# JunkyByte/easy_ViTPose

Hardware: NVIDIA H100
Metric: person-crops/sec ViT-B 256x192 bf16 (higher is better)
Workload: dtype bf16

## Files before the change

easy_vitpose_b200/csrc/engine.cu:

```cuda
#include <cuda.h>
#include <cuda_runtime.h>

#include <algorithm>
#include <cmath>
#include <cstdarg>
#include <cstdio>
#include <cstdlib>
#include <cstring>
#include <map>
#include <mutex>
#include <string>
#include <vector>

#include "../../include/vitpose_b200.h"
#include "attention.cuh"
#include "chain.cuh"
#include "decode.cuh"
#include "draw.cuh"
#include "expert_gemm.cuh"
#include "gemm.cuh"
#include "pointwise.cuh"
#include "preprocess.cuh"
#include "qkv_attention.cuh"
#include "track.cuh"
// ... 81 lines not shown
static cudaError_t launch_k(void (*kern)(KArgs...), dim3 grid, dim3 block, size_t smem, cudaStream_t st, Args&&... args) {
  cudaLaunchConfig_t cfg;
  memset(&cfg, 0, sizeof(cfg));
  cfg.gridDim = grid; cfg.blockDim = block; cfg.dynamicSmemBytes = smem; cfg.stream = st;
  cudaLaunchAttribute at[1];
  at[0].id = cudaLaunchAttributeProgrammaticStreamSerialization;
  at[0].val.programmaticStreamSerializationAllowed = 1;
  cfg.attrs = at; cfg.numAttrs = g_pdl ? 1 : 0;
  return cudaLaunchKernelEx(&cfg, kern, std::forward<Args>(args)...);
}

constexpr int kMaxDevices = 64;
struct DeviceState {
  int sms = 0;
  bool attn_attr = false;
  unsigned gemm_attr = 0;
  unsigned expert_attr = 0;
};
static DeviceState g_devs[kMaxDevices];
static DeviceState* cur_dev() {
  int d = 0;
  if (cudaGetDevice(&d) != cudaSuccess || d < 0 || d >= kMaxDevices) d = 0;
  return &g_devs[d];
}
static int num_sms() { return cur_dev()->sms; }


constexpr int gemm_slot(int bn, int epi) {
  return (epi == EPI_BF16_GELU_ERF ? 3 : epi) * 5 + (bn == 256 ? 0 : bn == 128 ? 1 : bn == 144 ? 2 : bn == 32 ? 3 : 4);
}
static_assert(gemm_slot(192, EPI_F32_ADD) < 32, "gemm_attr has 32 bits");

template <int BN, int EPI>
static int gemm_launch_t(const CUtensorMap& ta, const CUtensorMap& tw, const CUtensorMap& tout, const GemmParams& p, cudaStream_t st) {
  using Cfg = GemmCfg<BN, EPI>;
  auto kern = gemm_bf16_wgmma<BN, EPI>;
  DeviceState* ds = cur_dev();
  if (ds->sms == 0) return fail(VPB_ERR_STATE, "gemm: device not initialised (device_check)");
  constexpr unsigned slot = 1u << gemm_slot(BN, EPI);
  if (!(ds->gemm_attr & slot)) {
    CU_TRY(cudaFuncSetAttribute(kern, cudaFuncAttributeMaxDynamicSharedMemorySize, Cfg::SMEM_BYTES));
    ds->gemm_attr |= slot;
  }
  const bool deconv = (EPI == EPI_BF16_RELU_UP);
  const int num_m = deconv ? p.M / (p.up_tr * p.up_tw) : (p.M + GEMM_BM - 1) / GEMM_BM;
  const int tiles = num_m * (deconv ? 4 : (p.N + BN - 1) / BN);
  const int grid = tiles < ds->sms ? tiles : ds->sms;
  CU_TRY(launch_k(kern, dim3(grid), dim3(GEMM_THREADS), Cfg::SMEM_BYTES, st, ta, tw, tout, p));
  return VPB_OK;
}
static int gemm_launch(int bn, int epi, const CUtensorMap& ta, const CUtensorMap& tw, const CUtensorMap& tout, const GemmParams& p,
                       cudaStream_t st) {
  if (p.K % GEMM_BK != 0 || p.K <= 0) return fail(VPB_ERR_ARG, "gemm: K=%d must be a positive multiple of 64", p.K);
  if (epi_uses_tma(epi) && (p.N % (epi == EPI_F32_ADD ? 32 : 64) != 0 || p.bias == nullptr))
    return fail(VPB_ERR_ARG, "gemm: TMA epilogue wants N %% 64 == 0 (N %% 32 == 0 for the fp32 one) and a bias");
#define VPB_CASE(BN_, EPI_) \
  if (bn == BN_ && epi == EPI_) return gemm_launch_t<BN_, EPI_>(ta, tw, tout, p, st);
  VPB_CASE(256, EPI_BF16) VPB_CASE(192, EPI_BF16) VPB_CASE(128, EPI_BF16)
  VPB_CASE(256, EPI_BF16_GELU) VPB_CASE(192, EPI_BF16_GELU) VPB_CASE(128, EPI_BF16_GELU)
  VPB_CASE(256, EPI_BF16_GELU_ERF) VPB_CASE(192, EPI_BF16_GELU_ERF) VPB_CASE(128, EPI_BF16_GELU_ERF)
  VPB_CASE(256, EPI_F32_ADD) VPB_CASE(192, EPI_F32_ADD) VPB_CASE(128, EPI_F32_ADD)
  VPB_CASE(256, EPI_BF16_RELU_UP)
  VPB_CASE(32, EPI_F32_NCHW) VPB_CASE(144, EPI_F32_NCHW)
#undef VPB_CASE
  return fail(VPB_ERR_ARG, "gemm: no kernel for BN=%d epilogue=%d", bn, epi);
}

constexpr int kExpertWidths[5] = {192, 128, 96, 64, 32};
static int expert_width(int P) {
  for (int w : kExpertWidths)
    if (P % w == 0) return w;
  return 0;
}
template <int BN>
static int expert_launch_t(const CUtensorMap& ta, const CUtensorMap& tw, const ExpertParams& p, cudaStream_t st) {
  using Cfg = TileCfg<BN, false>;
  auto kern = gemm_expert_segments<BN>;
  DeviceState* ds = cur_dev();
  if (ds->sms == 0) return fail(VPB_ERR_STATE, "expert gemm: device not initialised (device_check)");
  constexpr unsigned slot = 1u << (BN / 32);
// ... 195 lines not shown
};
struct HeadW {
  int K = 0, n_final = 0;
  LinearW dc1, dc2, fin;
  CUtensorMap m_fin_w;
};
struct Segment { int head, count; };
static bool operator==(const Segment& a, const Segment& b) { return a.head == b.head && a.count == b.count; }
struct vpb_engine {
  vpb_config cfg;
  int D, depth, heads, K, maxB;
  int num_kheads = 1, P = 0, Kmax = 0, expert_bn = 0;
  std::vector<HeadW> hw;
  bool finalized = false;
  int stop_after = 0;
  Profiler prof;
  struct CachedGraph { bool mixed; std::vector<Segment> segs; bool affine; cudaGraphExec_t exec; unsigned long long used; };
  std::vector<CachedGraph> graph_cache;
  unsigned long long graph_clock = 0;
  bool use_graph = true;
  bool l2_persist = true;
  size_t l2_window_bytes = 0;
  std::vector<cudaStream_t> l2_streams;
  float* g_kpts = nullptr;
  int32_t *g_idx = nullptr, *g_org = nullptr, *g_offs = nullptr;
  float* g_cs = nullptr;
  double* mat_stage = nullptr;
  float* cs_stage = nullptr;
  int32_t *pp_org = nullptr, *pp_offs = nullptr, *pp_status = nullptr;
  uint8_t* frame_stage[2] = {nullptr, nullptr};
  size_t frame_cap[2] = {0, 0};
  int32_t* bbox_stage[2] = {nullptr, nullptr};
  bool flip = false, flip_heads = false;
// ... 699 lines not shown
      else fuse_ln(p, e->lnf_g, e->lnf_b);
      e->prof.begin(KC_GEMM_FC2, st);
      int bn;
      const CUtensorMap* wm;
      VPB_TRY(pick_tile(b.fc2, M, &bn, &wm));
      p.rmw = resid_rmw(e->resid_rmw);
      VPB_TRY(gemm_launch(bn, EPI_F32_ADD, e->m_hid, *wm, e->o_x, p, st));
      e->prof.end(st);
    }
    if (stop == 8) return VPB_OK;
  }
  if (stop == 9) return VPB_OK;
  return standalone_ln(e->lnf_g, e->lnf_b);
}

static int head(vpb_engine* e, int B, float* d_heat, cudaStream_t st, int j = 0, int c0 = 0, int ch_stride = 0) {
  const int D = e->D;
  const int stop = e->stop_after;
  const HeadW& h = e->hw[j];
  CUtensorMap feat = e->m_feat_nhwc, d1 = e->m_d1_nhwc, d2 = e->m_d2;
  if (c0 > 0) {
    VPB_TRY(make_map_nhwc(&feat, e->xn + static_cast<size_t>(c0) * 192 * D, B, 16, 12, D, 8, 12));
    VPB_TRY(make_map_nhwc(&d1, e->d1 + static_cast<size_t>(c0) * 768 * 256, B, 32, 24, 256, 16, 8));
    VPB_TRY(make_map(&d2, e->d2 + static_cast<size_t>(c0) * 3072 * 256, static_cast<uint64_t>(B) * 3072, 256, 256, 128));
  }
  {
    GemmParams p = gp(B * 192, 256, 4 * D, h.dc1.b, e->d1 + static_cast<size_t>(c0) * 768 * 256, 256);
    p.up_h = 16; p.up_w = 12; p.up_tr = 8; p.up_tw = 12; p.up_c = D;
    e->prof.begin(KC_GEMM_DECONV, st);
    VPB_TRY(gemm_launch(256, EPI_BF16_RELU_UP, feat, *h.dc1.tile_map(256), e->m_xn, p, st));
    e->prof.end(st);
  }
  if (stop == 11) return VPB_OK;
  {
    GemmParams p = gp(B * 768, 256, 1024, h.dc2.b, e->d2 + static_cast<size_t>(c0) * 3072 * 256, 256);
    p.up_h = 32; p.up_w = 24; p.up_tr = 16; p.up_tw = 8; p.up_c = 256;
    e->prof.begin(KC_GEMM_DECONV, st);
    VPB_TRY(gemm_launch(256, EPI_BF16_RELU_UP, d1, *h.dc2.tile_map(256), e->m_xn, p, st));
    e->prof.end(st);
  }
  if (stop == 12) return VPB_OK;
  {
    GemmParams p = gp(B * 3072, h.n_final, 256, h.fin.b, d_heat, 0);
    p.n_valid = h.K; p.pix = 3072; p.ch_stride = ch_stride;
    e->prof.begin(KC_GEMM_FINAL, st);
    VPB_TRY(gemm_launch(h.n_final, EPI_F32_NCHW, d2, h.m_fin_w, d2, p, st));
    e->prof.end(st);
  }
  return VPB_OK;
}

static int apply_l2_policy(vpb_engine* e, cudaStream_t st) {
  if (!e->l2_persist || e->l2_window_bytes == 0) return VPB_OK;
  for (cudaStream_t s : e->l2_streams) if (s == st) return VPB_OK;
  cudaStreamAttrValue v;
// ... 73 lines not shown
  if (e->flip && 2 * batch > e->maxB)
    return fail(VPB_ERR_ARG, "batch %d: with flip test on a call takes at most max_batch / 2 = %d crops (max_batch=%d)", batch, e->maxB / 2, e->maxB);
  return VPB_OK;
}

extern "C" int vpb_forward(vpb_engine* e, const float* d_crops, int32_t batch, float* d_heatmaps, void* stream) {
  VPB_TRY(check_ready(e, batch));
  DeviceGuard dev_guard(e);
  if (!d_crops || !d_heatmaps) return fail(VPB_ERR_ARG, "vpb_forward: null pointer");
  cudaStream_t st = static_cast<cudaStream_t>(stream);
  VPB_TRY(apply_l2_policy(e, st));
  WsScope ws(e, st);
  VPB_TRY(ws.begin(batch));
  VPB_TRY(patch_gather(e, d_crops, batch, batch, st));
  VPB_TRY(backbone(e, batch, st));
  if (!(e->stop_after && e->stop_after <= 10)) VPB_TRY(head(e, batch, d_heatmaps, st));
  return ws.end();
}

extern "C" int vpb_forward_features(vpb_engine* e, const float* d_crops, int32_t batch, float* d_features, void* stream) {
  VPB_TRY(check_ready(e, batch));
  DeviceGuard dev_guard(e);
  if (!d_crops || !d_features) return fail(VPB_ERR_ARG, "vpb_forward_features: null pointer");
  cudaStream_t st = static_cast<cudaStream_t>(stream);
  WsScope ws(e, st);
  VPB_TRY(ws.begin(batch));
  VPB_TRY(patch_gather(e, d_crops, batch, batch, st));
  VPB_TRY(backbone(e, batch, st));
  const long long tot = static_cast<long long>(batch) * e->D * 192;
  tokens_to_nchw<<<cdiv(tot, 256), 256, 0, st>>>(e->xn, d_features, batch, e->D);
  CU_TRY(cudaGetLastError());
// ... 14 lines not shown
}
extern "C" int vpb_decode(const float* d_heatmaps, int32_t n, int32_t k, const int32_t* d_org_wh, float* d_kpts, int32_t* d_idx,
                          int32_t wrap_batch, void* stream) {
  return decode_launch(d_heatmaps, n, k, d_org_wh, nullptr, d_kpts, d_idx, wrap_batch, stream);
}
extern "C" int vpb_head(vpb_engine* e, const float* d_features, int32_t batch, float* d_heatmaps, void* stream) {
  VPB_TRY(check_ready(e, batch));
  DeviceGuard dev_guard(e);
  if (!d_features || !d_heatmaps) return fail(VPB_ERR_ARG, "vpb_head: null pointer");
  cudaStream_t st = static_cast<cudaStream_t>(stream);
  const long long tot = static_cast<long long>(batch) * e->D * 192;
  WsScope ws(e, st);
  VPB_TRY(ws.begin(0));
  nchw_to_tokens<<<cdiv(tot, 256), 256, 0, st>>>(d_features, e->xn, batch, e->D);
  CU_TRY(cudaGetLastError());
  VPB_TRY(head(e, batch, d_heatmaps, st));
  return ws.end();
}
extern "C" int vpb_flip_back(const float* d_in, int32_t n, int32_t k, const int32_t* d_perm, int32_t shift, float* d_out, void* stream) {
  if (!d_in || !d_out || !d_perm || d_in == d_out) return fail(VPB_ERR_ARG, "vpb_flip_back: null or aliased pointers");
  if (n < 0 || k < 1) return fail(VPB_ERR_ARG, "vpb_flip_back: n=%d k=%d", n, k);
  if (n == 0) return VPB_OK;
  const long long tot = static_cast<long long>(n) * k * 3072;
  flip_back_heatmaps<<<cdiv(tot, 256), 256, 0, static_cast<cudaStream_t>(stream)>>>(d_in, d_out, d_perm, n, k, shift);
  CU_TRY(cudaGetLastError());
  return VPB_OK;
}
static bool gauss_taps(int ksize, GaussTaps& tp) {
  if (ksize < 1 || ksize > 2 * MAX_RADIUS + 1 || ksize % 2 == 0) return false;
  const int r = ksize / 2;
  if (ksize <= 9) {
// ... 85 lines not shown
  return out;
}

static int row_stride(const vpb_engine* e, bool mixed) { return mixed ? e->Kmax : e->K; }

static int heads_enqueue(vpb_engine* e, const Source* src, const std::vector<Segment>& segs, int n, int kstride, const int32_t* d_org_wh,
                         const int32_t* d_offs_yx, const float* d_cs, float* d_kpts, int32_t* d_idx, float* heat, cudaStream_t st) {
  const std::vector<Segment> msegs = model_segments(e, segs);
  const int nb = model_crops(e, n);
  if (src) VPB_TRY(gather(e, *src, n, nb, st));
  VPB_TRY(backbone(e, nb, st, (msegs.size() == 1 && msegs[0].head == 0) ? nullptr : &msegs));
  if (e->stop_after && e->stop_after <= 10) return VPB_OK;
  float* raw = e->flip ? e->heat : heat;
  int c0 = 0;
  for (const Segment& sg : msegs) {
    VPB_TRY(head(e, sg.count, raw + static_cast<size_t>(c0) * kstride * 3072, st, sg.head, c0, kstride));
    c0 += sg.count;
  }
  if (e->stop_after) return VPB_OK;
  c0 = 0;
  for (const Segment& sg : segs) {
    const size_t m0 = static_cast<size_t>(c0) * kstride * 3072;
    const int K = e->hw[sg.head].K;
    if (e->flip) VPB_TRY(flip_average(e, raw + m0, sg.count, K, e->flip_perm + perm_offset(e, sg.head), kstride, n, heat + m0, st));
    DecodeParams p;
    p.heatmaps = heat + m0; p.org_wh = d_cs ? nullptr : d_org_wh + 2 * c0; p.offs_yx = (d_offs_yx && !d_cs) ? d_offs_yx + 2 * c0 : nullptr;
    p.kpts = d_kpts + static_cast<size_t>(c0) * kstride * 3; p.idx = d_idx ? d_idx + static_cast<size_t>(c0) * kstride : nullptr;
    p.n = sg.count; p.k = K; p.kstride = kstride;
    p.wrap_batch = d_cs ? 1 : 0;
    p.cs32 = d_cs ? d_cs + 4 * c0 : nullptr;
    e->prof.begin(KC_DECODE, st);
// ... 19 lines not shown
  return VPB_OK;
}

static_assert(2 * VPB_MAX_SEGMENTS <= EXPERT_MAX_SEGMENTS, "a flip-test call's crops and mirror images fit the expert GEMM's table");
constexpr size_t kMaxMixedGraphs = 16;

static void drop_graphs(vpb_engine* e) {
  for (auto& g : e->graph_cache) if (g.exec) cudaGraphExecDestroy(g.exec);
  e->graph_cache.clear();
}

static int heads_core_locked(vpb_engine* e, const Source& src, const std::vector<Segment>& segs, bool mixed, int n, const int32_t* d_org_wh,
                             const int32_t* d_offs_yx, float* d_kpts, int32_t* d_idx, float* d_heatmaps, cudaStream_t st) {
  float* heat = d_heatmaps ? d_heatmaps : e->heat;
  const int ks = row_stride(e, mixed);
  if (!e->use_graph || e->prof.on || e->stop_after || st == nullptr || stream_is_capturing(st))
    return heads_enqueue(e, &src, segs, n, ks, d_org_wh, d_offs_yx, src.cs, d_kpts, d_idx, heat, st);
  const bool affine = src.cs != nullptr;
  vpb_engine::CachedGraph* g = nullptr;
  for (auto& c : e->graph_cache)
    if (c.mixed == mixed && c.segs == segs && c.affine == affine) g = &c;
  if (!g) {
    if (mixed) {
      auto lru = e->graph_cache.end();
      size_t count = 0;
      for (auto it = e->graph_cache.begin(); it != e->graph_cache.end(); ++it)
        if (it->mixed) {
          ++count;
          if (lru == e->graph_cache.end() || it->used < lru->used) lru = it;
        }
// ... 899 lines not shown
  if (!e || !entries || !captured) return fail(VPB_ERR_ARG, "vpb_cached_graphs: null argument");
  *entries = *captured = 0;
  for (const auto& g : e->graph_cache)
    if (g.mixed == (mixed != 0)) { ++*entries; *captured += g.exec != nullptr; }
  return VPB_OK;
}
extern "C" int64_t vpb_device_bytes(const vpb_engine* e) {
  if (!e) return -1;
  size_t b = e->alloc_bytes;
  for (int s = 0; s < 2; ++s) b += e->frame_cap[s] ? e->frame_cap[s] + 256 : 0;
  return static_cast<int64_t>(b);
}

extern "C" int vpb_kernel_launches(const vpb_engine* e, int32_t batch) {
  if (!e) return -1;
  if (e->use_chain && model_crops(e, batch) >= e->chain_min_batch && !e->ln_fused)
    return 1 + (1 + e->depth) + e->depth + 2 + 1 + 1 + (e->flip ? 1 : 0);
  return 2 + e->depth * (fuse_qkv_attention(e, model_crops(e, batch)) ? 4 : 5) + 2 + 1 + 1 +
         (e->ln_fused ? 0 : e->ln_in_gemm ? 1 : 2 * e->depth + 1) + (e->flip ? 1 : 0);
}

static int poison_workspace(vpb_engine* e) {
  if (!e->finalized) return fail(VPB_ERR_STATE, "poison: not finalized");
  DeviceGuard dev_guard(e);
  CU_TRY(cudaDeviceSynchronize());
  const size_t B = e->maxB, M = B * 192, D = e->D, K = e->Kmax, bf = sizeof(__nv_bfloat16), f = sizeof(float);
  const std::pair<void*, size_t> bufs[] = {
      {e->patch_rows, M * 768 * bf}, {e->x, M * D * f}, {e->xn, M * D * bf}, {e->qkv, M * 3 * D * bf}, {e->attn, M * D * bf},
      {e->hid, M * 4 * D * bf}, {e->d1, B * 768 * 256 * bf}, {e->d2, B * 3072 * 256 * bf}, {e->heat, B * K * 3072 * f},
      {e->g_kpts, B * K * 3 * f}, {e->kpts[0], B * K * 3 * f}, {e->kpts[1], B * K * 3 * f},
      {e->crops_stage[0], B * 3 * 256 * 192 * f}, {e->crops_stage[1], B * 3 * 256 * 192 * f}, {e->g_cs, B * 4 * f}, {e->cs_stage, B * 4 * f}};
  for (const auto& b : bufs) CU_TRY(cudaMemset(b.first, 0xFF, b.second));
  CU_TRY(cudaDeviceSynchronize());
// ... 7 lines not shown
  else if (!strcmp(name, "profile")) e->prof.on = value != 0;
  else if (!strcmp(name, "pdl")) g_pdl = value != 0;
  else if (!strcmp(name, "graph")) e->use_graph = value != 0;
  else if (!strcmp(name, "chain") || !strcmp(name, "chain_min_batch") || !strcmp(name, "gelu_erf") || !strcmp(name, "ln_in_gemm") ||
           !strcmp(name, "resid_rmw") || !strcmp(name, "ln_ctl") || !strcmp(name, "ln_job_rows")) {
    if (!strcmp(name, "ln_job_rows") && value != 8 && value != 16) return fail(VPB_ERR_ARG, "ln_job_rows must be 8 or 16");
    if (!strcmp(name, "gelu_erf")) e->gelu_erf = value != 0;
    else if (!strcmp(name, "resid_rmw")) e->resid_rmw = value != 0;
    else if (!strcmp(name, "ln_ctl")) e->ln_ctl = value != 0;
    else if (!strcmp(name, "ln_job_rows")) e->ln_job_rows = value;
    else if (!strcmp(name, "ln_in_gemm")) e->ln_in_gemm = value != 0;
    else if (!strcmp(name, "chain")) e->use_chain = value != 0;
    else e->chain_min_batch = value;
    drop_graphs(e);
  }
  else if (!strcmp(name, "ln_fused")) {
    e->ln_fused = value != 0;
    drop_graphs(e);
  }
  else return fail(VPB_ERR_ARG, "unknown option %s", name);
  return VPB_OK;
}

extern "C" int vpb_set_flip_test(vpb_engine* e, const int32_t* h_perm, int32_t k, int32_t shift) {
  if (!e) return fail(VPB_ERR_ARG, "vpb_set_flip_test: null engine");
  if (!e->finalized) return fail(VPB_ERR_STATE, "not finalized");
  if (e->num_kheads > 1) return fail(VPB_ERR_STATE, "vpb_set_flip_test: not supported on an engine with %d heads", e->num_kheads);
  if (h_perm) {
    if (k != e->K) return fail(VPB_ERR_ARG, "vpb_set_flip_test: permutation of %d keypoints, the engine has %d", k, e->K);
    for (int i = 0; i < k; ++i)
// ... 48 lines not shown
  return VPB_OK;
}

extern "C" int vpb_read_buffer(vpb_engine* e, const char* name, void* host_dst, int64_t bytes) {
  if (!e || !name || !host_dst) return fail(VPB_ERR_ARG, "vpb_read_buffer: null argument");
  if (!e->finalized) return fail(VPB_ERR_STATE, "not finalized");
  const void* src = nullptr;
  const std::string n(name);
  if (n == "patch_rows") src = e->patch_rows;
  else if (n == "x") src = e->x;
  else if (n == "xn") src = e->xn;
  else if (n == "qkv") src = e->qkv;
  else if (n == "attn") src = e->attn;
  else if (n == "hid") src = e->hid;
  else if (n == "d1") src = e->d1;
  else if (n == "d2") src = e->d2;
  else if (n == "heat") src = e->heat;
  else return fail(VPB_ERR_ARG, "unknown buffer %s", name);
  CU_TRY(cudaDeviceSynchronize());
  CU_TRY(cudaMemcpy(host_dst, src, bytes, cudaMemcpyDeviceToHost));
  return VPB_OK;
}

extern "C" int vpb_gemm(const void* d_a, const void* d_w, const float* d_bias, void* d_out, int32_t m, int32_t n, int32_t k,
                        int32_t epilogue, const float* d_resid, int32_t resid_mod, int32_t aux0, int32_t aux1, int32_t aux2,
                        int32_t aux3, void* stream) {
  int dev = 0;
  CU_TRY(cudaGetDevice(&dev));
  VPB_TRY(device_check(dev));
  if (!d_a || !d_w || !d_out) return fail(VPB_ERR_ARG, "vpb_gemm: null pointer");
  int bn;
// ... 54 lines not shown
```

easy_vitpose_b200/csrc/gemm.cuh:

```cuda
#pragma once
#include <cuda.h>

#include "ptx.cuh"
#include "wgmma.cuh"

namespace vpb {

enum Epilogue : int {
  EPI_BF16 = 0,
  EPI_BF16_GELU = 1,
  EPI_BF16_RELU_UP = 2,
  EPI_F32_NCHW = 4,
  EPI_F32_ADD = 5,
  EPI_BF16_GELU_ERF = 6,
};

struct GemmParams {
  int M, N, K;
  const float* bias;
  void* out;
  int ldc;
  int n_valid;
  int pix;
  int ch_stride;
  int up_h, up_w;
  int up_tr, up_tw;
  int up_c;
  const float* ln_gamma;
  const float* ln_beta;
  __nv_bfloat16* ln_out;
  int* ln_counters;
  float ln_eps;
  int rmw;
  int stages_limit;
  int dbg_flags;
  long long* dbg;
};

constexpr int GEMM_BM = 128;
constexpr int GEMM_BK = 64;
constexpr int GEMM_THREADS = 384;
constexpr int GEMM_CONSUMER_WARPS = 8;
constexpr int GEMM_STAGE_TILE = 8192;
constexpr int GEMM_BAR_EPI = 1;

__host__ __device__ constexpr bool epi_uses_tma(int epi) { return epi == EPI_BF16 || epi == EPI_BF16_GELU || epi == EPI_F32_ADD || epi == EPI_BF16_GELU_ERF; }

template <int BN, bool STAGED>
struct TileCfg {
  static constexpr int A_BYTES = GEMM_BM * GEMM_BK * 2;
  static constexpr int B_BYTES = BN * GEMM_BK * 2;
  static constexpr int STAGE_BYTES = A_BYTES + B_BYTES;
  static constexpr int STAGING = STAGED ? 4 * GEMM_STAGE_TILE : 0;
  static constexpr int STAGES_RAW = (227 * 1024 - 2048 - STAGING) / STAGE_BYTES;
  static constexpr int STAGES = STAGES_RAW > 8 ? 8 : STAGES_RAW;
  static constexpr int SMEM_BYTES = STAGES * STAGE_BYTES + STAGING + 1024  + 256 ;
  static_assert(B_BYTES % 1024 == 0, "W tiles must keep 1024-byte alignment of the ring");
  static_assert(BN % 16 == 0 && BN >= 16 && BN <= 256, "wgmma N");
  static_assert(!STAGED || BN % 64 == 0, "TMA epilogues stage 64 bf16 / 32 f32 columns at a time");
  static_assert(STAGES >= 3, "ring too shallow");
};
template <int BN, int EPI>
using GemmCfg = TileCfg<BN, epi_uses_tma(EPI)>;

__device__ __forceinline__ float gelu_erf_as(float x) { return 0.5f * x * (1.0f + erf_as(x * 0.70710678118654752440f)); }
#ifdef VPB_GELU_ERF
__device__ __forceinline__ float gelu_fast(float x) { return gelu_erf_as(x); }
#else
__device__ __forceinline__ float gelu_fast(float x) { return gelu_tanh_fit(x); }
#endif

struct RingPos {
  int stage = 0;
  uint32_t phase = 0;
  __device__ __forceinline__ void next(int stages) { if (++stage == stages) { stage = 0; phase ^= 1; } }
};

__device__ __forceinline__ void ring_wait_slot(uint64_t* empty_bar, const RingPos& rp) { mbar_wait(&empty_bar[rp.stage], rp.phase ^ 1); }
// ... 120 lines not shown
#pragma unroll
  for (int o = 16; o > 0; o >>= 1) q += __shfl_xor_sync(0xffffffffu, q, o);
  const float rstd = rsqrtf(q * (1.0f / D) + eps);
  uint2* yr = reinterpret_cast<uint2*>(yrow);
#pragma unroll
  for (int i = 0; i < V; ++i) {
    const float4 g = __ldg(reinterpret_cast<const float4*>(gamma) + i * 32 + lane);
    const float4 b = __ldg(reinterpret_cast<const float4*>(beta) + i * 32 + lane);
    uint2 o;
    o.x = pack_bf16(v[i].x * rstd * g.x + b.x, v[i].y * rstd * g.y + b.y);
    o.y = pack_bf16(v[i].z * rstd * g.z + b.z, v[i].w * rstd * g.w + b.w);
    yr[i * 32 + lane] = o;
  }
}

template <int BN, int EPI>
__global__ void __launch_bounds__(GEMM_THREADS, 1)
gemm_bf16_wgmma(const __grid_constant__ CUtensorMap tmap_a, const __grid_constant__ CUtensorMap tmap_w,
                const __grid_constant__ CUtensorMap tmap_out, const GemmParams p) {
  using Cfg = GemmCfg<BN, EPI>;
  extern __shared__ uint8_t smem_raw[];
  uint8_t* smem = reinterpret_cast<uint8_t*>((reinterpret_cast<uintptr_t>(smem_raw) + 1023) & ~uintptr_t(1023));
  uint8_t* ring = smem;
  uint8_t* staging = smem + Cfg::STAGES * Cfg::STAGE_BYTES;
  uint64_t* full_bar = reinterpret_cast<uint64_t*>(staging + Cfg::STAGING);
  uint64_t* empty_bar = full_bar + Cfg::STAGES;
  volatile int* ln_flag = reinterpret_cast<volatile int*>(empty_bar + Cfg::STAGES);

  const int warp = __shfl_sync(0xffffffffu, threadIdx.x >> 5, 0);
  const int lane = threadIdx.x & 31;
  constexpr bool kDeconv = (EPI == EPI_BF16_RELU_UP);
  const int up_pos = kDeconv ? p.up_tr * p.up_tw : GEMM_BM;
  const int num_m = kDeconv ? p.M / up_pos : (p.M + GEMM_BM - 1) / GEMM_BM;
  const int num_n = kDeconv ? 4 : (p.N + BN - 1) / BN;
  const int num_tiles = num_m * num_n;
  const int num_kb = p.K / GEMM_BK;
  const int num_stages = (p.stages_limit > 0 && p.stages_limit < Cfg::STAGES) ? p.stages_limit : Cfg::STAGES;
  auto tile_mn = [&](int tile, int& mt, int& nb) {
    if (p.dbg_flags & 4) { mt = tile % num_m; nb = tile / num_m; }
    else { mt = tile / num_n; nb = tile % num_n; }
  };

  const long long t_cta0 = (p.dbg && threadIdx.x == 0) ? clock64() : 0;
  if (threadIdx.x == 0) {
    tma_prefetch_desc(&tmap_a);
    tma_prefetch_desc(&tmap_w);
    if constexpr (epi_uses_tma(EPI)) tma_prefetch_desc(&tmap_out);
    for (int s = 0; s < Cfg::STAGES; ++s) {
      mbar_init(&full_bar[s], 1);
      mbar_init(&empty_bar[s], GEMM_CONSUMER_WARPS);
    }
    fence_mbar_init();
  }
  __syncthreads();
  pdl_launch_dependents();
  pdl_wait();

  if (warp >= GEMM_CONSUMER_WARPS) {
    setmaxnreg_dec<40>();
    if (warp != GEMM_CONSUMER_WARPS) return;
    RingPos rp;
    long long t_wait = 0;
    const long long t_begin = p.dbg ? clock64() : 0;
    const int tiles_x = kDeconv ? p.up_w / p.up_tw : 1;
    const int tiles_per_img = kDeconv ? (p.up_h / p.up_tr) * tiles_x : 1;
    const int kb_per_tap = kDeconv ? p.up_c / GEMM_BK : 1;
    for (int tile = blockIdx.x; tile < num_tiles; tile += gridDim.x) {
      int mt, nb;
      tile_mn(tile, mt, nb);
      const int m0 = (p.dbg_flags & 1) ? 0 : mt * GEMM_BM;
      const int n0 = (p.dbg_flags & 2) ? 0 : nb * BN;
      for (int kb = 0; kb < num_kb; ++kb) {
        const long long w0 = p.dbg ? clock64() : 0;
        ring_wait_slot(empty_bar, rp);
        if (p.dbg) t_wait += clock64() - w0;
        uint8_t* sa = ring + rp.stage * Cfg::STAGE_BYTES;
        if (elect_one()) {
          if constexpr (kDeconv) {
            const int tap = kb / kb_per_tap, c0 = (kb % kb_per_tap) * GEMM_BK;
            const int py = nb >> 1, px = nb & 1, iy = tap >> 1, ix = tap & 1;
            const int dy = py ? (iy ? 0 : 1) : (iy ? -1 : 0);
// ... 16 lines not shown
    setmaxnreg_inc<232>();
    const int wg = warp >> 2;
    const int tid = threadIdx.x & 127;
    const int wq = warp & 3;
    uint8_t* stiles = staging + wg * 2 * GEMM_STAGE_TILE;
    RingPos rp;
    int sfirst = 0;
    long long t_full = 0;
    const long long t_begin = p.dbg ? clock64() : 0;
    float acc[BN / 2];
    for (int tile = blockIdx.x; tile < num_tiles; tile += gridDim.x) {
      int mt, nb;
      tile_mn(tile, mt, nb);
      const int m0 = mt * GEMM_BM;
      const int n0 = kDeconv ? 0 : nb * BN;
      tile_mainloop<BN>(acc, ring, Cfg::STAGE_BYTES, full_bar, empty_bar, num_kb, num_stages, rp, wg, lane,
                        (p.dbg && threadIdx.x == 0) ? &t_full : nullptr);
      const int row0 = m0 + 64 * wg;

      if constexpr (epi_uses_tma(EPI)) {
        if (EPI == EPI_F32_ADD && p.rmw) epilogue_f32_rmw<BN>(acc, n0, row0, p.M, p.bias, reinterpret_cast<float*>(p.out), p.ldc, tid);
        else {
          epilogue_tma<BN, EPI>(acc, n0, row0, p.N, p.bias, stiles, wg, tid, &tmap_out, sfirst);
          sfirst ^= (BN / (EPI == EPI_F32_ADD ? 32 : 64)) & 1;
        }
      } else {
        const int cq = 2 * (lane & 3);
#pragma unroll
        for (int h = 0; h < 2; ++h) {
          const int r = 64 * wg + 16 * wq + (lane >> 2) + 8 * h;
          if constexpr (EPI == EPI_BF16_RELU_UP) {
            if (r >= up_pos || mt >= num_m) continue;
            const int tiles_x = p.up_w / p.up_tw;
            const int tiles_per_img = (p.up_h / p.up_tr) * tiles_x;
            const int b = mt / tiles_per_img, ti = mt % tiles_per_img;
// ... 69 lines not shown
```

easy_vitpose_b200/csrc/wgmma.cuh:

```cuda
#pragma once
#include <stdint.h>

namespace vpb {

__device__ __forceinline__ void wgmma_fence() { asm volatile("wgmma.fence.sync.aligned;" ::: "memory"); }
__device__ __forceinline__ void wgmma_commit() { asm volatile("wgmma.commit_group.sync.aligned;" ::: "memory"); }
template <int N>
__device__ __forceinline__ void wgmma_wait() { asm volatile("wgmma.wait_group.sync.aligned %0;" ::"n"(N) : "memory"); }
template <int N>
__device__ __forceinline__ void wgmma_fence_regs(float (&d)[N]) {
#pragma unroll
  for (int i = 0; i < N; ++i) asm volatile("" : "+f"(d[i])::"memory");
}

__device__ __forceinline__ void wgmma_ss_n32(float (&d)[16], uint64_t adesc, uint64_t bdesc, int accumulate) {
  asm volatile(
      "{\n\t.reg .pred p;\n\tsetp.ne.b32 p, %18, 0;\n\t"
      "wgmma.mma_async.sync.aligned.m64n32k16.f32.bf16.bf16 {%0, %1, %2, %3, %4, %5, %6, %7, %8, %9, %10, %11, %12, %13, %14, %15}, %16, %17, p, 1, 1, 0, 0;\n\t}"
      : "+f"(d[0]), "+f"(d[1]), "+f"(d[2]), "+f"(d[3]), "+f"(d[4]), "+f"(d[5]), "+f"(d[6]), "+f"(d[7]), "+f"(d[8]), "+f"(d[9]), "+f"(d[10]), "+f"(d[11]), "+f"(d[12]), "+f"(d[13]), "+f"(d[14]), "+f"(d[15])
      : "l"(adesc), "l"(bdesc), "r"(accumulate));
}
__device__ __forceinline__ void wgmma_ss_n64(float (&d)[32], uint64_t adesc, uint64_t bdesc, int accumulate) {
  asm volatile(
      "{\n\t.reg .pred p;\n\tsetp.ne.b32 p, %34, 0;\n\t"
// ... 55 lines not shown
__device__ __forceinline__ void wgmma_rs_n32(float (&d)[16], const uint32_t (&a)[4], uint64_t bdesc, int accumulate) {
  asm volatile(
      "{\n\t.reg .pred p;\n\tsetp.ne.b32 p, %21, 0;\n\t"
      "wgmma.mma_async.sync.aligned.m64n32k16.f32.bf16.bf16 {%0, %1, %2, %3, %4, %5, %6, %7, %8, %9, %10, %11, %12, %13, %14, %15}, {%16, %17, %18, %19}, %20, p, 1, 1, %22;\n\t}"
      : "+f"(d[0]), "+f"(d[1]), "+f"(d[2]), "+f"(d[3]), "+f"(d[4]), "+f"(d[5]), "+f"(d[6]), "+f"(d[7]), "+f"(d[8]), "+f"(d[9]), "+f"(d[10]), "+f"(d[11]), "+f"(d[12]), "+f"(d[13]), "+f"(d[14]), "+f"(d[15])
      : "r"(a[0]), "r"(a[1]), "r"(a[2]), "r"(a[3]), "l"(bdesc), "r"(accumulate), "n"(TRANS_B));
}
template <int TRANS_B>
__device__ __forceinline__ void wgmma_rs_n64(float (&d)[32], const uint32_t (&a)[4], uint64_t bdesc, int accumulate) {
  asm volatile(
      "{\n\t.reg .pred p;\n\tsetp.ne.b32 p, %37, 0;\n\t"
      "wgmma.mma_async.sync.aligned.m64n64k16.f32.bf16.bf16 {%0, %1, %2, %3, %4, %5, %6, %7, %8, %9, %10, %11, %12, %13, %14, %15, %16, %17, %18, %19, %20, %21, %22, %23, %24, %25, %26, %27, %28, %29, %30, %31}, {%32, %33, %34, %35}, %36, p, 1, 1, %38;\n\t}"
      : "+f"(d[0]), "+f"(d[1]), "+f"(d[2]), "+f"(d[3]), "+f"(d[4]), "+f"(d[5]), "+f"(d[6]), "+f"(d[7]), "+f"(d[8]), "+f"(d[9]), "+f"(d[10]), "+f"(d[11]), "+f"(d[12]), "+f"(d[13]), "+f"(d[14]), "+f"(d[15]), "+f"(d[16]), "+f"(d[17]), "+f"(d[18]), "+f"(d[19]), "+f"(d[20]), "+f"(d[21]), "+f"(d[22]), "+f"(d[23]), "+f"(d[24]), "+f"(d[25]), "+f"(d[26]), "+f"(d[27]), "+f"(d[28]), "+f"(d[29]), "+f"(d[30]), "+f"(d[31])
      : "r"(a[0]), "r"(a[1]), "r"(a[2]), "r"(a[3]), "l"(bdesc), "r"(accumulate), "n"(TRANS_B));
}
template <int N>
__device__ __forceinline__ void wgmma_ss(float (&d)[N / 2], uint64_t adesc, uint64_t bdesc, int accumulate) {
  if constexpr (N == 32) wgmma_ss_n32(d, adesc, bdesc, accumulate);
  else if constexpr (N == 64) wgmma_ss_n64(d, adesc, bdesc, accumulate);
  else if constexpr (N == 96) wgmma_ss_n96(d, adesc, bdesc, accumulate);
  else if constexpr (N == 128) wgmma_ss_n128(d, adesc, bdesc, accumulate);
  else if constexpr (N == 144) wgmma_ss_n144(d, adesc, bdesc, accumulate);
  else if constexpr (N == 192) wgmma_ss_n192(d, adesc, bdesc, accumulate);
  else if constexpr (N == 240) wgmma_ss_n240(d, adesc, bdesc, accumulate);
  else if constexpr (N == 256) wgmma_ss_n256(d, adesc, bdesc, accumulate);
  else static_assert(N == 0, "no wgmma wrapper for this N (tools/gen_wgmma.py)");
}

}
```

Before: 11900.

## Fuse second deconv with final 1x1 head conv via register-operand wgmma

Adds a fused epilogue to the deconv GEMM. It applies bias and ReLU, packs the 256 deconv channels to bf16 in registers, and multiplies them by the final 1x1 conv weights held in shared memory with register-A wgmma. The result is written straight to the NCHW heatmaps, so the bf16 d2 intermediate (B*3072*256) is never written or re-read and one kernel launch goes away. The cost is shared memory taken from the pipeline ring for the head weights, plus a larger accumulator register footprint in the epilogue. Debug reads of d2 now recompute it lazily. The fusion is enabled by default for non-chained batches of at least 16 crops.

```diff
diff --git a/easy_vitpose_b200/csrc/engine.cu b/easy_vitpose_b200/csrc/engine.cu
--- a/easy_vitpose_b200/csrc/engine.cu
+++ b/easy_vitpose_b200/csrc/engine.cu
@@ -119,7 +119,7 @@
 struct DeviceState {
   int sms = 0;
   bool attn_attr = false;
-  unsigned gemm_attr = 0;
+  uint64_t gemm_attr = 0;
   unsigned expert_attr = 0;
 };
 static DeviceState g_devs[kMaxDevices];
@@ -132,22 +132,23 @@
 
 
 constexpr int gemm_slot(int bn, int epi) {
-  return (epi == EPI_BF16_GELU_ERF ? 3 : epi) * 5 + (bn == 256 ? 0 : bn == 128 ? 1 : bn == 144 ? 2 : bn == 32 ? 3 : 4);
-}
-static_assert(gemm_slot(192, EPI_F32_ADD) < 32, "gemm_attr has 32 bits");
-
-template <int BN, int EPI>
+  return (epi == EPI_BF16_GELU_ERF ? 3 : epi == EPI_F32_NCHW_HEAD ? 7 : epi) * 5 + (bn == 256 ? 0 : bn == 128 ? 1 : bn == 144 ? 2 : bn == 32 ? 3 : 4);
+}
+static_assert(gemm_slot(192, EPI_F32_ADD) < 30 && gemm_slot(144, EPI_F32_NCHW_HEAD) > 31 && gemm_slot(192, EPI_F32_NCHW_HEAD) < 64,
+              "gemm_attr bits");
+
+template <int BN, int EPI, int NF = 0>
 static int gemm_launch_t(const CUtensorMap& ta, const CUtensorMap& tw, const CUtensorMap& tout, const GemmParams& p, cudaStream_t st) {
-  using Cfg = GemmCfg<BN, EPI>;
-  auto kern = gemm_bf16_wgmma<BN, EPI>;
+  using Cfg = GemmCfg<BN, EPI, NF>;
+  auto kern = gemm_bf16_wgmma<BN, EPI, NF>;
   DeviceState* ds = cur_dev();
   if (ds->sms == 0) return fail(VPB_ERR_STATE, "gemm: device not initialised (device_check)");
-  constexpr unsigned slot = 1u << gemm_slot(BN, EPI);
+  constexpr uint64_t slot = 1ull << gemm_slot(EPI == EPI_F32_NCHW_HEAD ? NF : BN, EPI);
   if (!(ds->gemm_attr & slot)) {
     CU_TRY(cudaFuncSetAttribute(kern, cudaFuncAttributeMaxDynamicSharedMemorySize, Cfg::SMEM_BYTES));
     ds->gemm_attr |= slot;
   }
-  const bool deconv = (EPI == EPI_BF16_RELU_UP);
+  const bool deconv = (EPI == EPI_BF16_RELU_UP || EPI == EPI_F32_NCHW_HEAD);
   const int num_m = deconv ? p.M / (p.up_tr * p.up_tw) : (p.M + GEMM_BM - 1) / GEMM_BM;
   const int tiles = num_m * (deconv ? 4 : (p.N + BN - 1) / BN);
   const int grid = tiles < ds->sms ? tiles : ds->sms;
@@ -169,6 +170,14 @@
   VPB_CASE(32, EPI_F32_NCHW) VPB_CASE(144, EPI_F32_NCHW)
 #undef VPB_CASE
   return fail(VPB_ERR_ARG, "gemm: no kernel for BN=%d epilogue=%d", bn, epi);
+}
+static int deconv_head_launch(int n_final, const CUtensorMap& ta, const CUtensorMap& tw, const CUtensorMap& tfin, const GemmParams& p,
+                              cudaStream_t st) {
+  if (p.N != 256 || p.bias == nullptr || p.bias2 == nullptr)
+    return fail(VPB_ERR_ARG, "deconv head: N=%d: wants 256 deconv channels and both biases", p.N);
+  if (n_final == 32) return gemm_launch_t<256, EPI_F32_NCHW_HEAD, 32>(ta, tw, tfin, p, st);
+  if (n_final == 144) return gemm_launch_t<256, EPI_F32_NCHW_HEAD, 144>(ta, tw, tfin, p, st);
+  return fail(VPB_ERR_ARG, "deconv head: no kernel for n_final=%d", n_final);
 }
 
 constexpr int kExpertWidths[5] = {192, 128, 96, 64, 32};
@@ -394,9 +403,12 @@
   std::vector<HeadW> hw;
   bool finalized = false;
   int stop_after = 0;
+  int head_form = 0;
   Profiler prof;
   struct CachedGraph { bool mixed; std::vector<Segment> segs; bool affine; cudaGraphExec_t exec; unsigned long long used; };
   std::vector<CachedGraph> graph_cache;
+  std::vector<Segment> d2_segs;
+  bool d2_stale = false;
   unsigned long long graph_clock = 0;
   bool use_graph = true;
   bool l2_persist = true;
@@ -1126,7 +1138,26 @@
   return standalone_ln(e->lnf_g, e->lnf_b);
 }
 
-static int head(vpb_engine* e, int B, float* d_heat, cudaStream_t st, int j = 0, int c0 = 0, int ch_stride = 0) {
+static int deconv2_store(vpb_engine* e, int B, cudaStream_t st, int j, int c0, const CUtensorMap& d1) {
+  GemmParams p = gp(B * 768, 256, 1024, e->hw[j].dc2.b, e->d2 + static_cast<size_t>(c0) * 3072 * 256, 256);
+  p.up_h = 32; p.up_w = 24; p.up_tr = 16; p.up_tw = 8; p.up_c = 256;
+  return gemm_launch(256, EPI_BF16_RELU_UP, d1, *e->hw[j].dc2.tile_map(256), e->m_xn, p, st);
+}
+
+static void note_head_pass(vpb_engine* e, const std::vector<Segment>& msegs, bool fused) {
+  e->d2_segs = msegs;
+  e->d2_stale = fused;
+}
+
+constexpr int kFuseHeadMinCrops = 16;
+static bool fuse_head(const vpb_engine* e, int crops) {
+  if (e->stop_after) return false;
+  if (e->head_form) return e->head_form == 1;
+  const bool chained = e->use_chain && crops >= e->chain_min_batch && !e->ln_fused;
+  return !chained && crops >= kFuseHeadMinCrops;
+}
+
+static int head(vpb_engine* e, int B, float* d_heat, cudaStream_t st, bool fuse, int j = 0, int c0 = 0, int ch_stride = 0) {
   const int D = e->D;
   const int stop = e->stop_after;
   const HeadW& h = e->hw[j];
@@ -1134,7 +1165,7 @@
   if (c0 > 0) {
     VPB_TRY(make_map_nhwc(&feat, e->xn + static_cast<size_t>(c0) * 192 * D, B, 16, 12, D, 8, 12));
     VPB_TRY(make_map_nhwc(&d1, e->d1 + static_cast<size_t>(c0) * 768 * 256, B, 32, 24, 256, 16, 8));
-    VPB_TRY(make_map(&d2, e->d2 + static_cast<size_t>(c0) * 3072 * 256, static_cast<uint64_t>(B) * 3072, 256, 256, 128));
+    if (!fuse) VPB_TRY(make_map(&d2, e->d2 + static_cast<size_t>(c0) * 3072 * 256, static_cast<uint64_t>(B) * 3072, 256, 256, 128));
   }
   {
     GemmParams p = gp(B * 192, 256, 4 * D, h.dc1.b, e->d1 + static_cast<size_t>(c0) * 768 * 256, 256);
@@ -1144,13 +1175,18 @@
     e->prof.end(st);
   }
   if (stop == 11) return VPB_OK;
-  {
-    GemmParams p = gp(B * 768, 256, 1024, h.dc2.b, e->d2 + static_cast<size_t>(c0) * 3072 * 256, 256);
+  if (fuse) {
+    GemmParams p = gp(B * 768, 256, 1024, h.dc2.b, d_heat, 0);
     p.up_h = 32; p.up_w = 24; p.up_tr = 16; p.up_tw = 8; p.up_c = 256;
+    p.n_valid = h.K; p.pix = 3072; p.ch_stride = ch_stride; p.bias2 = h.fin.b;
     e->prof.begin(KC_GEMM_DECONV, st);
-    VPB_TRY(gemm_launch(256, EPI_BF16_RELU_UP, d1, *h.dc2.tile_map(256), e->m_xn, p, st));
+    VPB_TRY(deconv_head_launch(h.n_final, d1, *h.dc2.tile_map(256), h.m_fin_w, p, st));
     e->prof.end(st);
-  }
+    return VPB_OK;
+  }
+  e->prof.begin(KC_GEMM_DECONV, st);
+  VPB_TRY(deconv2_store(e, B, st, j, c0, d1));
+  e->prof.end(st);
   if (stop == 12) return VPB_OK;
   {
     GemmParams p = gp(B * 3072, h.n_final, 256, h.fin.b, d_heat, 0);
@@ -1254,7 +1290,9 @@
   VPB_TRY(ws.begin(batch));
   VPB_TRY(patch_gather(e, d_crops, batch, batch, st));
   VPB_TRY(backbone(e, batch, st));
-  if (!(e->stop_after && e->stop_after <= 10)) VPB_TRY(head(e, batch, d_heatmaps, st));
+  const bool fuse = fuse_head(e, batch);
+  if (!(e->stop_after && e->stop_after <= 10)) VPB_TRY(head(e, batch, d_heatmaps, st, fuse));
+  note_head_pass(e, {{0, batch}}, fuse);
   return ws.end();
 }
 
@@ -1299,7 +1337,9 @@
   VPB_TRY(ws.begin(0));
   nchw_to_tokens<<<cdiv(tot, 256), 256, 0, st>>>(d_features, e->xn, batch, e->D);
   CU_TRY(cudaGetLastError());
-  VPB_TRY(head(e, batch, d_heatmaps, st));
+  const bool fuse = fuse_head(e, batch);
+  VPB_TRY(head(e, batch, d_heatmaps, st, fuse));
+  note_head_pass(e, {{0, batch}}, fuse);
   return ws.end();
 }
 extern "C" int vpb_flip_back(const float* d_in, int32_t n, int32_t k, const int32_t* d_perm, int32_t shift, float* d_out, void* stream) {
@@ -1415,7 +1455,7 @@
   float* raw = e->flip ? e->heat : heat;
   int c0 = 0;
   for (const Segment& sg : msegs) {
-    VPB_TRY(head(e, sg.count, raw + static_cast<size_t>(c0) * kstride * 3072, st, sg.head, c0, kstride));
+    VPB_TRY(head(e, sg.count, raw + static_cast<size_t>(c0) * kstride * 3072, st, fuse_head(e, nb), sg.head, c0, kstride));
     c0 += sg.count;
   }
   if (e->stop_after) return VPB_OK;
@@ -1465,6 +1505,7 @@
                              const int32_t* d_offs_yx, float* d_kpts, int32_t* d_idx, float* d_heatmaps, cudaStream_t st) {
   float* heat = d_heatmaps ? d_heatmaps : e->heat;
   const int ks = row_stride(e, mixed);
+  note_head_pass(e, model_segments(e, segs), fuse_head(e, model_crops(e, n)));
   if (!e->use_graph || e->prof.on || e->stop_after || st == nullptr || stream_is_capturing(st))
     return heads_enqueue(e, &src, segs, n, ks, d_org_wh, d_offs_yx, src.cs, d_kpts, d_idx, heat, st);
   const bool affine = src.cs != nullptr;
@@ -2394,9 +2435,10 @@
 
 extern "C" int vpb_kernel_launches(const vpb_engine* e, int32_t batch) {
   if (!e) return -1;
+  const int fin = fuse_head(e, model_crops(e, batch)) ? 0 : 1;
   if (e->use_chain && model_crops(e, batch) >= e->chain_min_batch && !e->ln_fused)
-    return 1 + (1 + e->depth) + e->depth + 2 + 1 + 1 + (e->flip ? 1 : 0);
-  return 2 + e->depth * (fuse_qkv_attention(e, model_crops(e, batch)) ? 4 : 5) + 2 + 1 + 1 +
+    return 1 + (1 + e->depth) + e->depth + 2 + fin + 1 + (e->flip ? 1 : 0);
+  return 2 + e->depth * (fuse_qkv_attention(e, model_crops(e, batch)) ? 4 : 5) + 2 + fin + 1 +
          (e->ln_fused ? 0 : e->ln_in_gemm ? 1 : 2 * e->depth + 1) + (e->flip ? 1 : 0);
 }
 
@@ -2434,6 +2476,11 @@
     else e->chain_min_batch = value;
     drop_graphs(e);
   }
+  else if (!strcmp(name, "head_form")) {
+    if (value < 0 || value > 2) return fail(VPB_ERR_ARG, "head_form must be 0 (rule), 1 (fused) or 2 (three launches)");
+    e->head_form = value;
+    drop_graphs(e);
+  }
   else if (!strcmp(name, "ln_fused")) {
     e->ln_fused = value != 0;
     drop_graphs(e);
@@ -2512,7 +2559,21 @@
   else if (n == "attn") src = e->attn;
   else if (n == "hid") src = e->hid;
   else if (n == "d1") src = e->d1;
-  else if (n == "d2") src = e->d2;
+  else if (n == "d2") {
+    if (e->d2_stale) {
+      DeviceGuard dev_guard(e);
+      CU_TRY(cudaDeviceSynchronize());
+      int c0 = 0;
+      for (const Segment& sg : e->d2_segs) {
+        CUtensorMap d1 = e->m_d1_nhwc;
+        if (c0 > 0) VPB_TRY(make_map_nhwc(&d1, e->d1 + static_cast<size_t>(c0) * 768 * 256, sg.count, 32, 24, 256, 16, 8));
+        VPB_TRY(deconv2_store(e, sg.count, nullptr, sg.head, c0, d1));
+        c0 += sg.count;
+      }
+      e->d2_stale = false;
+    }
+    src = e->d2;
+  }
   else if (n == "heat") src = e->heat;
   else return fail(VPB_ERR_ARG, "unknown buffer %s", name);
   CU_TRY(cudaDeviceSynchronize());
diff --git a/easy_vitpose_b200/csrc/gemm.cuh b/easy_vitpose_b200/csrc/gemm.cuh
--- a/easy_vitpose_b200/csrc/gemm.cuh
+++ b/easy_vitpose_b200/csrc/gemm.cuh
@@ -13,6 +13,7 @@
   EPI_F32_NCHW = 4,
   EPI_F32_ADD = 5,
   EPI_BF16_GELU_ERF = 6,
+  EPI_F32_NCHW_HEAD = 7,
 };
 
 struct GemmParams {
@@ -26,6 +27,7 @@
   int up_h, up_w;
   int up_tr, up_tw;
   int up_c;
+  const float* bias2;
   const float* ln_gamma;
   const float* ln_beta;
   __nv_bfloat16* ln_out;
@@ -46,22 +48,24 @@
 
 __host__ __device__ constexpr bool epi_uses_tma(int epi) { return epi == EPI_BF16 || epi == EPI_BF16_GELU || epi == EPI_F32_ADD || epi == EPI_BF16_GELU_ERF; }
 
-template <int BN, bool STAGED>
+template <int BN, bool STAGED, int EXTRA_BYTES = 0>
 struct TileCfg {
+  static constexpr int EXTRA = EXTRA_BYTES;
   static constexpr int A_BYTES = GEMM_BM * GEMM_BK * 2;
   static constexpr int B_BYTES = BN * GEMM_BK * 2;
   static constexpr int STAGE_BYTES = A_BYTES + B_BYTES;
   static constexpr int STAGING = STAGED ? 4 * GEMM_STAGE_TILE : 0;
-  static constexpr int STAGES_RAW = (227 * 1024 - 2048 - STAGING) / STAGE_BYTES;
+  static constexpr int STAGES_RAW = (227 * 1024 - 2048 - STAGING - EXTRA) / STAGE_BYTES;
   static constexpr int STAGES = STAGES_RAW > 8 ? 8 : STAGES_RAW;
-  static constexpr int SMEM_BYTES = STAGES * STAGE_BYTES + STAGING + 1024  + 256 ;
+  static constexpr int SMEM_BYTES = STAGES * STAGE_BYTES + STAGING + EXTRA + 1024  + 256 ;
+  static_assert(EXTRA % 1024 == 0, "extra region keeps the 1024-byte alignment of the swizzled tiles");
   static_assert(B_BYTES % 1024 == 0, "W tiles must keep 1024-byte alignment of the ring");
   static_assert(BN % 16 == 0 && BN >= 16 && BN <= 256, "wgmma N");
   static_assert(!STAGED || BN % 64 == 0, "TMA epilogues stage 64 bf16 / 32 f32 columns at a time");
   static_assert(STAGES >= 3, "ring too shallow");
 };
-template <int BN, int EPI>
-using GemmCfg = TileCfg<BN, epi_uses_tma(EPI)>;
+template <int BN, int EPI, int NF = 0>
+using GemmCfg = TileCfg<BN, epi_uses_tma(EPI), EPI == EPI_F32_NCHW_HEAD ? NF * 256 * 2 : 0>;
 
 __device__ __forceinline__ float gelu_erf_as(float x) { return 0.5f * x * (1.0f + erf_as(x * 0.70710678118654752440f)); }
 #ifdef VPB_GELU_ERF
@@ -212,22 +216,76 @@
   }
 }
 
-template <int BN, int EPI>
+template <int NF>
+__device__ __forceinline__ void epilogue_head(const float (&acc)[128], const GemmParams& p, uint32_t w_smem, uint64_t* w_bar, int mt,
+                                              int nb, int wg, int tid) {
+  const int lane = tid & 31, wq = tid >> 5;
+  const int cq = 2 * (lane & 3);
+  uint32_t a[64];
+#pragma unroll
+  for (int j = 0; j < 32; ++j) {
+    const float2 b2 = __ldg(reinterpret_cast<const float2*>(p.bias + 8 * j + cq));
+    a[2 * j] = pack_bf16(relu_keep_nan(acc[4 * j] + b2.x), relu_keep_nan(acc[4 * j + 1] + b2.y));
+    a[2 * j + 1] = pack_bf16(relu_keep_nan(acc[4 * j + 2] + b2.x), relu_keep_nan(acc[4 * j + 3] + b2.y));
+  }
+  float d[NF / 2];
+#pragma unroll
+  for (int i = 0; i < NF / 2; ++i) d[i] = 0.f;
+  mbar_wait(w_bar, 0);
+  wgmma_fence();
+#pragma unroll
+  for (int s = 0; s < 16; ++s) {
+    const uint32_t f[4] = {a[4 * s], a[4 * s + 1], a[4 * s + 2], a[4 * s + 3]};
+    const uint64_t bd = wgmma_desc<128>(w_smem + (s >> 2) * NF * 128) + 2 * (s & 3);
+    if constexpr (NF == 32) wgmma_rs_n32<0>(d, f, bd, s != 0);
+    else wgmma_rs_n144<0>(d, f, bd, s != 0);
+  }
+  wgmma_commit();
+  wgmma_wait<0>();
+  wgmma_fence_regs(d);
+  const int tiles_x = p.up_w / p.up_tw;
+  const int tiles_per_img = (p.up_h / p.up_tr) * tiles_x;
+  const int b = mt / tiles_per_img, ti = mt % tiles_per_img;
+  const int up_pos = p.up_tr * p.up_tw;
+  const float* bias2 = p.bias2 + cq;
+#pragma unroll
+  for (int h = 0; h < 2; ++h) {
+    const int r = 64 * wg + 16 * wq + (lane >> 2) + 8 * h;
+    if (r >= up_pos) continue;
+    const int y = (ti / tiles_x) * p.up_tr + r / p.up_tw, x = (ti % tiles_x) * p.up_tw + r % p.up_tw;
+    const int pix = (2 * y + (nb >> 1)) * (2 * p.up_w) + (2 * x + (nb & 1));
+    float* o = reinterpret_cast<float*>(p.out) + (static_cast<size_t>(b) * (p.ch_stride ? p.ch_stride : p.n_valid)) * p.pix + pix;
+#pragma unroll
+    for (int j = 0; j < NF / 8; ++j) {
+      const int n = 8 * j + cq;
+      const float2 b2 = __ldg(reinterpret_cast<const float2*>(bias2 + 8 * j));
+      const float v0 = d[4 * j + 2 * h] + b2.x, v1 = d[4 * j + 2 * h + 1] + b2.y;
+      if (n < p.n_valid) o[static_cast<size_t>(n) * p.pix] = v0;
+      if (n + 1 < p.n_valid) o[static_cast<size_t>(n + 1) * p.pix] = v1;
+    }
+  }
+}
+
+template <int BN, int EPI, int NF = 0>
 __global__ void __launch_bounds__(GEMM_THREADS, 1)
 gemm_bf16_wgmma(const __grid_constant__ CUtensorMap tmap_a, const __grid_constant__ CUtensorMap tmap_w,
                 const __grid_constant__ CUtensorMap tmap_out, const GemmParams p) {
-  using Cfg = GemmCfg<BN, EPI>;
+  using Cfg = GemmCfg<BN, EPI, NF>;
   extern __shared__ uint8_t smem_raw[];
   uint8_t* smem = reinterpret_cast<uint8_t*>((reinterpret_cast<uintptr_t>(smem_raw) + 1023) & ~uintptr_t(1023));
   uint8_t* ring = smem;
   uint8_t* staging = smem + Cfg::STAGES * Cfg::STAGE_BYTES;
-  uint64_t* full_bar = reinterpret_cast<uint64_t*>(staging + Cfg::STAGING);
+  uint8_t* head_w = staging + Cfg::STAGING;
+  uint64_t* full_bar = reinterpret_cast<uint64_t*>(head_w + Cfg::EXTRA);
   uint64_t* empty_bar = full_bar + Cfg::STAGES;
   volatile int* ln_flag = reinterpret_cast<volatile int*>(empty_bar + Cfg::STAGES);
+  uint64_t* head_bar = empty_bar + Cfg::STAGES + 1;
 
   const int warp = __shfl_sync(0xffffffffu, threadIdx.x >> 5, 0);
   const int lane = threadIdx.x & 31;
-  constexpr bool kDeconv = (EPI == EPI_BF16_RELU_UP);
+  constexpr bool kHead = (EPI == EPI_F32_NCHW_HEAD);
+  constexpr bool kDeconv = (EPI == EPI_BF16_RELU_UP) || kHead;
+  static_assert(!kHead || (BN == 256 && (NF == 32 || NF == 144)), "the fused head takes all 256 deconv channels; n_final 32 or 144");
   const int up_pos = kDeconv ? p.up_tr * p.up_tw : GEMM_BM;
   const int num_m = kDeconv ? p.M / up_pos : (p.M + GEMM_BM - 1) / GEMM_BM;
   const int num_n = kDeconv ? 4 : (p.N + BN - 1) / BN;
@@ -243,11 +301,12 @@
   if (threadIdx.x == 0) {
     tma_prefetch_desc(&tmap_a);
     tma_prefetch_desc(&tmap_w);
-    if constexpr (epi_uses_tma(EPI)) tma_prefetch_desc(&tmap_out);
+    if constexpr (epi_uses_tma(EPI) || kHead) tma_prefetch_desc(&tmap_out);
     for (int s = 0; s < Cfg::STAGES; ++s) {
       mbar_init(&full_bar[s], 1);
       mbar_init(&empty_bar[s], GEMM_CONSUMER_WARPS);
     }
+    if constexpr (kHead) mbar_init(head_bar, 1);
     fence_mbar_init();
   }
   __syncthreads();
@@ -263,6 +322,14 @@
     const int tiles_x = kDeconv ? p.up_w / p.up_tw : 1;
     const int tiles_per_img = kDeconv ? (p.up_h / p.up_tr) * tiles_x : 1;
     const int kb_per_tap = kDeconv ? p.up_c / GEMM_BK : 1;
+    if constexpr (kHead) {
+      if (elect_one()) {
+        mbar_expect_tx(head_bar, NF * 256 * 2);
+#pragma unroll
+        for (int c = 0; c < 4; ++c) tma_load_2d(head_w + c * NF * 128, &tmap_out, head_bar, c * GEMM_BK, 0);
+      }
+      __syncwarp();
+    }
     for (int tile = blockIdx.x; tile < num_tiles; tile += gridDim.x) {
       int mt, nb;
       tile_mn(tile, mt, nb);
@@ -309,11 +376,17 @@
       tile_mn(tile, mt, nb);
       const int m0 = mt * GEMM_BM;
       const int n0 = kDeconv ? 0 : nb * BN;
+      if constexpr (kHead) {
+#pragma unroll
+        for (int i = 0; i < BN / 2; ++i) acc[i] = 0.f;
+      }
       tile_mainloop<BN>(acc, ring, Cfg::STAGE_BYTES, full_bar, empty_bar, num_kb, num_stages, rp, wg, lane,
                         (p.dbg && threadIdx.x == 0) ? &t_full : nullptr);
       const int row0 = m0 + 64 * wg;
 
-      if constexpr (epi_uses_tma(EPI)) {
+      if constexpr (kHead) {
+        epilogue_head<NF>(acc, p, smem_u32(head_w), head_bar, mt, nb, wg, tid);
+      } else if constexpr (epi_uses_tma(EPI)) {
         if (EPI == EPI_F32_ADD && p.rmw) epilogue_f32_rmw<BN>(acc, n0, row0, p.M, p.bias, reinterpret_cast<float*>(p.out), p.ldc, tid);
         else {
           epilogue_tma<BN, EPI>(acc, n0, row0, p.N, p.bias, stiles, wg, tid, &tmap_out, sfirst);
diff --git a/easy_vitpose_b200/csrc/wgmma.cuh b/easy_vitpose_b200/csrc/wgmma.cuh
--- a/easy_vitpose_b200/csrc/wgmma.cuh
+++ b/easy_vitpose_b200/csrc/wgmma.cuh
@@ -93,6 +93,14 @@
       : "+f"(d[0]), "+f"(d[1]), "+f"(d[2]), "+f"(d[3]), "+f"(d[4]), "+f"(d[5]), "+f"(d[6]), "+f"(d[7]), "+f"(d[8]), "+f"(d[9]), "+f"(d[10]), "+f"(d[11]), "+f"(d[12]), "+f"(d[13]), "+f"(d[14]), "+f"(d[15]), "+f"(d[16]), "+f"(d[17]), "+f"(d[18]), "+f"(d[19]), "+f"(d[20]), "+f"(d[21]), "+f"(d[22]), "+f"(d[23]), "+f"(d[24]), "+f"(d[25]), "+f"(d[26]), "+f"(d[27]), "+f"(d[28]), "+f"(d[29]), "+f"(d[30]), "+f"(d[31])
       : "r"(a[0]), "r"(a[1]), "r"(a[2]), "r"(a[3]), "l"(bdesc), "r"(accumulate), "n"(TRANS_B));
 }
+template <int TRANS_B>
+__device__ __forceinline__ void wgmma_rs_n144(float (&d)[72], const uint32_t (&a)[4], uint64_t bdesc, int accumulate) {
+  asm volatile(
+      "{\n\t.reg .pred p;\n\tsetp.ne.b32 p, %77, 0;\n\t"
+      "wgmma.mma_async.sync.aligned.m64n144k16.f32.bf16.bf16 {%0, %1, %2, %3, %4, %5, %6, %7, %8, %9, %10, %11, %12, %13, %14, %15, %16, %17, %18, %19, %20, %21, %22, %23, %24, %25, %26, %27, %28, %29, %30, %31, %32, %33, %34, %35, %36, %37, %38, %39, %40, %41, %42, %43, %44, %45, %46, %47, %48, %49, %50, %51, %52, %53, %54, %55, %56, %57, %58, %59, %60, %61, %62, %63, %64, %65, %66, %67, %68, %69, %70, %71}, {%72, %73, %74, %75}, %76, p, 1, 1, %78;\n\t}"
+      : "+f"(d[0]), "+f"(d[1]), "+f"(d[2]), "+f"(d[3]), "+f"(d[4]), "+f"(d[5]), "+f"(d[6]), "+f"(d[7]), "+f"(d[8]), "+f"(d[9]), "+f"(d[10]), "+f"(d[11]), "+f"(d[12]), "+f"(d[13]), "+f"(d[14]), "+f"(d[15]), "+f"(d[16]), "+f"(d[17]), "+f"(d[18]), "+f"(d[19]), "+f"(d[20]), "+f"(d[21]), "+f"(d[22]), "+f"(d[23]), "+f"(d[24]), "+f"(d[25]), "+f"(d[26]), "+f"(d[27]), "+f"(d[28]), "+f"(d[29]), "+f"(d[30]), "+f"(d[31]), "+f"(d[32]), "+f"(d[33]), "+f"(d[34]), "+f"(d[35]), "+f"(d[36]), "+f"(d[37]), "+f"(d[38]), "+f"(d[39]), "+f"(d[40]), "+f"(d[41]), "+f"(d[42]), "+f"(d[43]), "+f"(d[44]), "+f"(d[45]), "+f"(d[46]), "+f"(d[47]), "+f"(d[48]), "+f"(d[49]), "+f"(d[50]), "+f"(d[51]), "+f"(d[52]), "+f"(d[53]), "+f"(d[54]), "+f"(d[55]), "+f"(d[56]), "+f"(d[57]), "+f"(d[58]), "+f"(d[59]), "+f"(d[60]), "+f"(d[61]), "+f"(d[62]), "+f"(d[63]), "+f"(d[64]), "+f"(d[65]), "+f"(d[66]), "+f"(d[67]), "+f"(d[68]), "+f"(d[69]), "+f"(d[70]), "+f"(d[71])
+      : "r"(a[0]), "r"(a[1]), "r"(a[2]), "r"(a[3]), "l"(bdesc), "r"(accumulate), "n"(TRANS_B));
+}
 template <int N>
 __device__ __forceinline__ void wgmma_ss(float (&d)[N / 2], uint64_t adesc, uint64_t bdesc, int accumulate) {
   if constexpr (N == 32) wgmma_ss_n32(d, adesc, bdesc, accumulate);
```

New measurement: 12100, median of 6. 1.02x the previous value.
